# kamisli-icpl/LLICTI

Measured on AMD Instinct MI355X. Metric: MPix/s encode+decode, higher is better.
Workload: dtype f32; 1 GPU; 24x768x512 uniform-noise RGB per GPU, container xauto15 -> xrans20, seed-1337 weights; BASELINE.json configs[2]; batch_per_gpu=24, height=512, width=768, container=xauto15, container_written=xrans20

## Files before the change

### llicti_amd/csrc/cdf.hpp

```cpp
#pragma once

__device__ __forceinline__ StageGeom stage_at(const StageGeom &s, const StageGeom *__restrict__ sv, int b)
{
    if (sv) return sv[b];
    StageGeom r = s;
    r.img_off = (long)b * 3 * s.plane;
    r.par_off = (long)b * LLICTI_PARAM_STRIDE * s.h * s.w;
    r.pair_off = (long)b * s.hc * s.wc;
    return r;
}

__device__ __forceinline__ void clr_range(const int32_t *mm, int clr, int &minv, int &maxv, int &shift)
{
    if (clr == 0) { minv = -127; maxv = 128; shift = 127; }
    else { minv = mm[clr - 1]; maxv = mm[2 + clr - 1]; shift = -minv; }
}

constexpr int kPairsThreads = 256;
__device__ __forceinline__ void cdf_pairs_body(const int16_t *__restrict__ planes, const float *__restrict__ params,
                                               const int32_t *__restrict__ minmax, const StageGeom &s, uint32_t *__restrict__ pairs)
{
    const int b = blockIdx.y;
    const int lane = threadIdx.x & 63, wave = threadIdx.x >> 6;
    const int np = s.h * s.w;
    const int p0 = (blockIdx.x * (blockDim.x >> 6) + wave) * 64;
    if (p0 >= np) return;
    const ParRow par = par_row(params + s.par_off, 0, np, min(p0 + lane, np - 1));
    const int p = p0 + lane;
    const int i = p / s.w, j = p - i * s.w;
    if (p >= np || i >= s.hc || j >= s.wc) return;
    const long n = (long)i * s.wc + j;
    const long off = s.img_off + ((long)(2 * i + s.oi) << s.lvl) * s.W + ((long)(2 * j + s.oj) << s.lvl);
    const int vy = planes[off], vco = planes[off + s.plane], vcg = planes[off + 2 * s.plane];
    const float yv = div255_exact((float)vy), cov = div255_exact((float)vco);
    const int32_t *mm = minmax + 4 * b;
#pragma unroll
    for (int clr = 0; clr < 3; ++clr) {
        int minv, maxv, shift;
        clr_range(mm, clr, minv, maxv, shift);
        const Grid gr = make_grid(minv, maxv);
        const int v = (clr == 0) ? vy : (clr == 1) ? vco : vcg;
        const int sym = v + shift;
        Mix m;
        mix_prepare(par, clr, yv, cov, m);
        const uint32_t lo = cdf_entry(m, gr, sym);
        const uint32_t hi1 = cdf_entry(m, gr, min(sym + 1, gr.Lp - 2));
        const uint32_t hi = (sym == gr.Lp - 2) ? 0u : hi1;
        pairs[(long)clr * s.pair_cs + s.pair_off + n] = (hi << 16) | lo;
    }
}
__global__ __launch_bounds__(kPairsThreads) void cdf_pairs_kernel(const int16_t *__restrict__ planes, const float *__restrict__ params,
                                                        const int32_t *__restrict__ minmax, StageGeom s, const StageGeom *__restrict__ sv,
                                                        uint32_t *__restrict__ pairs)
{
    cdf_pairs_body(planes, params, minmax, stage_at(s, sv, blockIdx.y), pairs);
}
struct PairsBands { const StageGeom *sv[3]; const float *params[3]; uint32_t *pairs[3]; };
__global__ __launch_bounds__(kPairsThreads) void cdf_pairs_bands_kernel(const int16_t *__restrict__ planes, PairsBands a,
                                                              const int32_t *__restrict__ minmax)
{
    const int band = blockIdx.z;
    cdf_pairs_body(planes, a.params[band], minmax, a.sv[band][blockIdx.y], a.pairs[band]);
}

__device__ __forceinline__ Comp row_component(const ParRow &par, const int16_t *__restrict__ planes, long off, long plane, int clr, int mi, float &w)
{
    float a0 = 0.0f, a1 = 0.0f, y = 0.0f, co = 0.0f;
    if (clr == 1) { a0 = par[48 + mi]; y = (float)planes[off] / 255.0f; }
    else if (clr == 2) { a0 = par[48 + 5 + mi]; a1 = par[48 + 10 + mi]; y = (float)planes[off] / 255.0f; co = (float)planes[off + plane] / 255.0f; }
    Comp c = mix_component(clr, par[5 * clr + mi], par[16 + 5 * clr + mi], par[32 + 5 * clr + mi], a0, a1, y, co, w);
    float ssum = w + dpp_row_shl(w, 1);
    ssum = ssum + dpp_row_shl(w, 2);
    ssum = ssum + dpp_row_shl(w, 3);
    ssum = ssum + dpp_row_shl(w, 4);
    c.wn = w / mix_weight_den(__int_as_float(__builtin_amdgcn_readfirstlane(__float_as_int(ssum))));
    return c;
}

constexpr int kTabWaves = 4;

__global__ __launch_bounds__(64 * kTabWaves) void cdf_table_kernel(const int16_t *__restrict__ planes, const float *__restrict__ params,
                                                                   const int32_t *__restrict__ minmax, StageGeom s, int clr,
                                                                   uint16_t *__restrict__ tables, int row_stride,
                                                                   int n0, int cnt, int cap_rows)
{
    const int b = blockIdx.y;
    const int nc = s.hc * s.wc;
    const int lane = threadIdx.x & 63;
    const int wave0 = __builtin_amdgcn_readfirstlane((int)(blockIdx.x * kTabWaves + (threadIdx.x >> 6)));
    const int nwaves = gridDim.x * kTabWaves;
    int minv, maxv, shift;
    clr_range(minmax + 4 * b, clr, minv, maxv, shift);
    const Grid gr = make_grid(minv, maxv);
    const int nblk = (row_stride + 63) >> 6;
    float pt[8];
#pragma unroll
    for (int k = 0; k < 8; ++k) pt[k] = sample_pt(gr, min(64 * k + lane, gr.Lp - 1));
    const float fmin = (float)minv;
    const long img = (long)b * 3 * s.plane;
    const int mi = min(lane, 4);

    constexpr int kTabRun = 8;
    const int n_end = min(nc, n0 + cnt);
    for (int nb = n0 + kTabRun * wave0; nb < n_end; nb += kTabRun * nwaves)
    for (int n = nb; n < min(nb + kTabRun, n_end); ++n) {
        const int i = n / s.wc, j = n - i * s.wc;
        const ParRow par = par_row(params, b, (long)s.h * s.w, (long)i * s.w + j);
        const long off = img + ((long)(2 * i + s.oi) << s.lvl) * s.W + ((long)(2 * j + s.oj) << s.lvl);
        float w;
        const Comp cm = row_component(par, planes, off, s.plane, clr, mi, w);
        const float mu = cm.mu, rsig = cm.rsig, wn = cm.wn;
        const float c = mu * 255.0f - fmin + 0.5f, hw = 9.8994949f * 255.0f * mix_sigma(par[5 * clr + mi]) + 2.0f;
        int lo = -1, hi = 1 << 20;
        if (c - hw > -1.0f && c - hw < 1e6f) lo = (int)(c - hw);
        if (c + hw > -1e6f && c + hw < 1e6f) hi = (int)(c + hw) + 1;
        if (!(c == c) || !(hw == hw)) { lo = -1; hi = 1 << 20; }
        float mu_[5], rs_[5], wn_[5];
        int lo_[5], hi_[5];
#pragma unroll
        for (int k = 0; k < 5; ++k) {
            mu_[k] = __int_as_float(__builtin_amdgcn_readlane(__float_as_int(mu), k));
            rs_[k] = __int_as_float(__builtin_amdgcn_readlane(__float_as_int(rsig), k));
            wn_[k] = __int_as_float(__builtin_amdgcn_readlane(__float_as_int(wn), k));
            lo_[k] = __builtin_amdgcn_readlane(lo, k);
            hi_[k] = __builtin_amdgcn_readlane(hi, k);
        }
        uint16_t *row = tables + ((long)b * cap_rows + (n - n0)) * row_stride;
#pragma unroll
        for (int k = 0; k < 8; ++k) {
            if (k < nblk) {
                const int e = 64 * k + lane;
                const int ec = min(e, gr.Lp - 1);
                const int bmin = (k == 0) ? -20 : 64 * k;
                const int bmax = (64 * k + 63 >= gr.Lp - 1) ? gr.Lp + 19 : 64 * k + 63;
                float acc = 0.0f;
#pragma unroll
                for (int m = 0; m < 5; ++m) {
                    float t;
                    if (bmax <= lo_[m]) t = 0.0f;
                    else if (bmin >= hi_[m]) t = wn_[m];
                    else {
                        const float z = (pt[k] - mu_[m]) * rs_[m];
                        t = wn_[m] * (0.5f * erfc_spec(kNegRsqrt2 * z));
                    }
                    acc = (m == 0) ? t : acc + t;
                }
                const uint32_t v = entry_from_sum(acc, gr.scale, ec);
                if (e < row_stride) row[e] = (uint16_t)((e < gr.Lp) ? v : 0xFFFFu);
            }
        }
    }
}


__global__ __launch_bounds__(64 * kTabWaves) void cdf_anchor_kernel(const int16_t *__restrict__ planes, const float *__restrict__ params,
                                                                    const int32_t *__restrict__ minmax, StageGeom s, int clr,
                                                                    uint8_t *__restrict__ rows, int n0, int cnt, int cap_rows)
{
    const int b = blockIdx.y;
    const int nc = s.hc * s.wc;
    const int lane = threadIdx.x & 63;
    const int wave0 = __builtin_amdgcn_readfirstlane((int)(blockIdx.x * kTabWaves + (threadIdx.x >> 6)));
    const int nwaves = gridDim.x * kTabWaves;
    int minv, maxv, shift;
    clr_range(minmax + 4 * b, clr, minv, maxv, shift);
    const Grid gr = make_grid(minv, maxv);
    const int ec = min(8 * lane, gr.Lp - 1);
    const float pt = sample_pt(gr, ec);
    const long img = (long)b * 3 * s.plane;
    const int mi = min(lane, 4);
    for (int n = n0 + wave0; n < min(nc, n0 + cnt); n += nwaves) {
        const int i = n / s.wc, j = n - i * s.wc;
        const ParRow par = par_row(params, b, (long)s.h * s.w, (long)i * s.w + j);
        const long off = img + ((long)(2 * i + s.oi) << s.lvl) * s.W + ((long)(2 * j + s.oj) << s.lvl);
        float w;
        const Comp cm = row_component(par, planes, off, s.plane, clr, mi, w);
        const float mu = cm.mu, rsig = cm.rsig, wn = cm.wn;
        float acc = 0.0f;
#pragma unroll
        for (int m = 0; m < 5; ++m) {
// ... 14 lines not shown
```

### llicti_amd/csrc/llicti_hip.hip

```cpp
#include <hip/hip_runtime.h>
#include <stdarg.h>
#include <stdint.h>
#include <stdio.h>
#include <stdlib.h>
#include <string.h>
#include <map>
#include <memory>
#include <string>
#include <tuple>
#include <type_traits>
#include <utility>
#include <vector>

#include "../../include/llicti_hip.h"
#include "numerics.hpp"

using namespace llicti;

#include "common.hpp"
#include "lift.hpp"
#include "likelihood.hpp"
#include "band_cnn.hpp"
#include "cdf.hpp"
#include "ac_coder.hpp"
// ... 890 lines not shown
    TensorNorm nm{};
    PlanDev *target = nullptr;
    uint8_t *target_ws = nullptr;
};

static int resolve_sink(DecodeSink &k, int B, const int *Hs, const int *Ws, int reduce, const int *rv = nullptr)
{
    switch (k.kind) {
    case DecodeSink::Interleaved: {
        std::vector<int> Hw(B), Ww(B);
        for (int b = 0; b < B; ++b) { const int r = rv ? rv[b] : reduce; Hw[b] = reduced_dim(Hs[b], r); Ww[b] = reduced_dim(Ws[b], r); }
        return resolve_pixels("decode_images_px", B, Hw.data(), Ww.data(), k.px.fmt, k.px.off, k.px.pitch, k.pix);
    }
    case DecodeSink::Tensor:
        return resolve_tensor("decode_images_tensor", B, Hs, Ws, reduce, k.tensor, k.wins, k.nm, rv);
    case DecodeSink::Resized:
        return resolve_resize("decode_images_tensor_resized", B, Hs, Ws, reduce, k.resize, k.wins, k.nm, rv);
    case DecodeSink::Views:
        return resolve_views("decode_images_tensor_views", B, Hs, Ws, reduce, k.views, k.groups, k.nm, rv);
    default:
        return 0;
    }
}

template <typename F> static void with_tensor_type(int dtype, F &&f)
{
    if (dtype == LLICTI_T_F32) f(float());
    else if (dtype == LLICTI_T_F16) f(_Float16());
    else f(bf16_bits());
}
template <typename S> static S arg_slice(const std::vector<uint32_t> &words, int k, int first, int n)
{
    S a;
    memset(&a, 0, sizeof a);
    memcpy(a.w, words.data() + (size_t)k * first, (size_t)k * n * sizeof(uint32_t));
    return a;
}

static int launch_sink(llicti_ctx *c, PlanDev *pd, const DecodeSink &k, uint8_t *ws, hipStream_t s, int reduce, const RvCall *rv = nullptr)
{
    const int *rtab = rv ? rv->d_r() : nullptr;
    const Plan &p = pd->p;
    const int B = p.B;
    const int16_t *planes = (const int16_t *)(ws + p.off_planes);
    const int32_t *status = (const int32_t *)(ws + p.off_status);
    const ImgGeo *d_img = pd->dev<ImgGeo>(p.d_img);
    if (k.kind == DecodeSink::Transcode) return 0;
    ProfSpan span(c, PROF_MISC, s);
    switch (k.kind) {
    case DecodeSink::Tensor: {
        const TensorArgs &t = k.tensor;
        const int gx = (int)std::min<long>(((long)t.Ho * ((t.Wo + 3) / 4) + 255) / 256, 1024);
        for (int b0 = 0; b0 < B; b0 += kTensorWinMax) {
            const int nb = std::min(kTensorWinMax, B - b0);
            const TensorWins tw = arg_slice<TensorWins>(k.wins, 1, b0, nb);
            with_tensor_type(t.dtype, [&](auto e) {
                using T = decltype(e);
                unlift_tensor_kernel<T><<<dim3(gx, nb), 256, 0, s>>>(planes, (T *)k.d_out, reduce, t.Ho, t.Wo, b0, tw, k.nm, status, kStatusHead, c->d_status,
                                                                    c->d_img_status, d_img, rtab);
            });
        }
        break;
    }
    case DecodeSink::Resized: {
        const ResizeArgs &t = k.resize;
        const int tiles_x = (t.Wo + kResizeTileW - 1) / kResizeTileW, tiles_y = (t.Ho + kResizeTileH - 1) / kResizeTileH;
        for (int b0 = 0; b0 < B; b0 += kResizeBoxMax) {
            const int nb = std::min(kResizeBoxMax, B - b0);
            const ResizeBoxes bx = arg_slice<ResizeBoxes>(k.wins, 2, b0, nb);
            with_tensor_type(t.dtype, [&](auto e) {
                using T = decltype(e);
                unlift_resize_tensor_kernel<T><<<dim3(tiles_x * tiles_y, nb), 256, 0, s>>>(planes, (T *)k.d_out, reduce, t.Ho, t.Wo, b0, tiles_x, t.antialias, bx, k.nm,
                                                                                          status, kStatusHead, c->d_status, c->d_img_status, d_img, rtab);
            });
        }
        break;
    }
    case DecodeSink::Views: {
        int latch_n = B;
        for (const ViewGroupOut &g : k.groups) {
            const int tiles_x = (g.Wo + kResizeTileW - 1) / kResizeTileW, tiles_y = (g.Ho + kResizeTileH - 1) / kResizeTileH;
            for (int v0 = 0; v0 < g.n; v0 += kViewMax) {
                const int nv = std::min(kViewMax, g.n - v0);
                const ViewSlice vs = arg_slice<ViewSlice>(g.words, 3, v0, nv);
                with_tensor_type(g.dtype, [&](auto e) {
                    using T = decltype(e);
                    unlift_views_tensor_kernel<T><<<dim3(tiles_x * tiles_y, nv), 256, 0, s>>>(planes, (T *)g.d_out, reduce, g.Ho, g.Wo, v0, tiles_x, g.antialias, vs, k.nm,
                                                                                             status, kStatusHead, c->d_status, c->d_img_status, d_img, latch_n, rtab);
                });
                latch_n = 0;
            }
        }
        break;
    }
    case DecodeSink::Interleaved: {
        const int gx = (int)std::min<long>(((rv ? rv->q.pix_units : p.pix_units) + 255) / 256, 1024);
        if (rv) unlift_px_kernel<<<dim3(gx, B), 256, 0, s>>>(planes, k.d_out, 0, status, kStatusHead, c->d_status, c->d_img_status, d_img, rv->d_red(), rv->d_pix(), rtab);
        else unlift_px_kernel<<<dim3(gx, B), 256, 0, s>>>(planes, k.d_out, reduce, status, kStatusHead, c->d_status, c->d_img_status, d_img,
                                                          reduce > 0 ? pd->dev<RedGeo>(p.d_red) : nullptr, pd->dev<PixGeo>(p.d_pix));
        break;
    }
    default:
        if (rv) {
            unlift_reduced_kernel<<<dim3((unsigned)((rv->q.max_rplane + 255) / 256), B), 256, 0, s>>>(planes, k.d_out, 0, status, kStatusHead, c->d_status,
                                                                                                      c->d_img_status, d_img, rv->d_red(), rtab);
        } else if (reduce > 0) {
            long max_rplane = 0;
            for (const RedGeo &rg : p.red) max_rplane = std::max(max_rplane, (long)rg.Hr * rg.Wr);
            unlift_reduced_kernel<<<dim3((unsigned)((max_rplane + 255) / 256), B), 256, 0, s>>>(planes, k.d_out, reduce, status, kStatusHead, c->d_status,
                                                                                                c->d_img_status, d_img, pd->dev<RedGeo>(p.d_red));
        } else {
            const int gx = (int)std::min<long>((p.max_plane + 255) / 256, 1024);
            unlift_kernel<<<dim3(gx, B), 256, 0, s>>>(planes, p.max_plane, k.d_out, status, kStatusHead, c->d_status, c->d_img_status, d_img);
        }
    }
    HIPCHK(hipGetLastError());
    return 0;
}

static int decode_stages(llicti_ctx *c, PlanDev *pd, const uint8_t *d_in, size_t in_stride, const int32_t *d_seg_len, uint8_t *ws, hipStream_t s, int reduce,
                         const DecodeSink &sink, const RvCall *rv = nullptr)
{
    const Plan &p = pd->p;
    const int B = p.B, M = p.M, Q = p.Q;
    int16_t *planes = (int16_t *)(ws + p.off_planes);
    float *fplanes = (float *)(ws + p.off_fplanes);
    int32_t *mm = (int32_t *)(ws + p.off_minmax);
    int32_t *status = (int32_t *)(ws + p.off_status);
    float *params = (float *)(ws + p.off_params);
    uint8_t *slots = ws + p.off_slots;
    uint8_t *tables = ws + p.off_tables;
    uint32_t *acstate = (uint32_t *)(ws + p.off_acstate);
    int32_t *slot_len = (int32_t *)(ws + p.off_slot_len);
    const ImgGeo *d_img = pd->dev<ImgGeo>(p.d_img);
    const Geom *d_geo = pd->dev<Geom>(p.d_geo);
    const StageGeom *d_sg = pd->dev<StageGeom>(p.d_sg);
    const long *d_rslot_off = pd->dev<long>(p.d_rslot_off);
    const StreamRef *d_sref = pd->dev<StreamRef>(p.d_sref);
    const int NS = p.nstreams;
    const TileRef *d_tiles = p.uniform ? nullptr : pd->dev<TileRef>(p.d_tiles);

    zero_words_kernel<<<(kStatusHead + B + 255) / 256, 256, 0, s>>>(status, kStatusHead + B);
    uint32_t *rstate = (uint32_t *)(ws + p.off_rstate);
    uint32_t *rpos = (uint32_t *)(ws + p.off_rpos);
    uint32_t *rtail = (uint32_t *)(ws + p.off_rtail);
    {
        ProfSpan span(c, PROF_MISC, s);
        header_read_kernel<<<B, 256, 0, s>>>(d_in, (long)in_stride, d_seg_len, d_img, planes, fplanes, mm, status);
        if (M == 0) {
            const int st0 = first_stage(p.nlev);
            unpack_kernel<<<dim3(LLICTI_NSTREAMS - st0, B), 256, 0, s>>>(d_in, (long)in_stride, d_seg_len, B, slots, pd->dev<long>(p.d_slot_off), pd->dev<int32_t>(p.d_slot_cap), slot_len, status, st0);
        } else {
            const StageGeom *sglv = d_sg + (size_t)(0 * 3 + 2) * B;
            rans_unpack_kernel<<<NS, 256, 0, s>>>(d_in, (long)in_stride, d_seg_len, d_sref, 2 + Q * RansGeo<1>::kPayBytes,
                                                  slots, d_rslot_off, p.rslot_cap, rpos, status, Q == 4 ? 4 : 2);
            if (Q == 4) rans_init_kernel<4><<<NS, 64, 0, s>>>(slots, d_rslot_off, d_sref, rstate, rpos, rtail, status, sglv);
            else if (Q == 2) rans_init_kernel<2><<<NS, 64, 0, s>>>(slots, d_rslot_off, d_sref, rstate, rpos, rtail, status, sglv);
            else rans_init_kernel<1><<<NS, 64, 0, s>>>(slots, d_rslot_off, d_sref, rstate, rpos, rtail, status, sglv);
        }
    }
    if (rv && M == 0) return fail(LLICTI_EINVAL, "decode_images: per-image reduces need rANS containers");
    for (int lvl = p.nlev - 1; lvl >= reduce; --lvl) {
        const Geom &g = p.geo[(size_t)lvl * B];
        const Geom *gv = (p.uniform && !rv) ? nullptr : d_geo + (size_t)lvl * B;
        const int NS = rv ? rv->q.s_n[lvl] : p.nstreams;
        const int *act = rv ? rv->dev<int>(rv->q.d_streams) + rv->q.s_off[lvl] : nullptr;
        if (NS == 0 && M > 0) continue;
        for (int band = 0; band < 3; ++band) {
            const TileRun *run = rv ? &rv->q.run[lvl * 3 + band] : &p.run[lvl * 3 + band];
            const TileRef *tl = rv ? rv->dev<TileRef>(rv->q.d_tiles) + run->off : d_tiles ? d_tiles + run->off : nullptr;
            if (int rc = launch_band_params(c, fplanes, g, band, params, s, gv, tl, run)) return rc;
            const StageGeom *sgv = d_sg + (size_t)(lvl * 3 + band) * B;
            if (M > 0) {
                const int last = (lvl == 0 && band == 2) ? 1 : 0;
                {
                ProfSpan span(c, PROF_RANS_STAGE, s);
                if (Q == 4) {
                    rans_decode_stage_lane_kernel<4><<<NS, 256, 0, s>>>(params, sgv, d_sref, slots, d_rslot_off, p.rslot_cap, rstate, rpos, rtail, planes, fplanes, mm, last, status, c->d_phi_lut, act);
                } else if (Q == 2) {
                    rans_decode_stage_pair_kernel<<<NS, 64 * kRansWaves, 0, s>>>(params, sgv, d_sref, c->d_phi_lut, slots, d_rslot_off, p.rslot_cap, rstate, rpos, rtail, planes, fplanes, mm, last, status, act);
                } else {
                    rans_decode_stage_kernel<<<NS, 64 * kRansWaves, 0, s>>>(params, sgv, d_sref, c->d_phi_lut, slots, d_rslot_off, p.rslot_cap, rstate, rpos, rtail, planes, fplanes, mm, last, status, act);
                }
                }
                if (last) {
                    ProfSpan span(c, PROF_RANS_TAIL, s);
                    if (Q == 4) rans_tail_kernel<4><<<NS, 64 * (1 + kTailAhead) * kTailChains<4>, 0, s>>>(params, sgv, d_sref, rstate, rpos, rtail, planes, fplanes, mm, status, slots, d_rslot_off, act);
                    else if (Q == 2) rans_tail_kernel<2><<<NS, 64 * (1 + kTailAhead), 0, s>>>(params, sgv, d_sref, rstate, rpos, rtail, planes, fplanes, mm, status, slots, d_rslot_off, act);
                    else rans_tail_kernel<1><<<NS, 64 * (1 + kTailAhead), 0, s>>>(params, sgv, d_sref, rstate, rpos, rtail, planes, fplanes, mm, status, slots, d_rslot_off, act);
                }
            }
            if (M == 0) {
                const StageGeom sg = make_stage(g, band);
                const long nc = (long)sg.hc * sg.wc;
                const int C = ac_chunks(nc);
                const long rows = ac_chunk_rows(nc);
                hipStream_t q[3] = { s, c->sub[1], c->sub[2] };
                if (C > 1) {
                    HIPCHK(hipEventRecord(c->ev_ac_band, s));
                    HIPCHK(hipStreamWaitEvent(q[1], c->ev_ac_band, 0));
                    HIPCHK(hipStreamWaitEvent(q[2], c->ev_ac_band, 0));
                }
                for (int ch = 0; ch < C; ++ch) {
                    const long n0 = (long)ch * rows, cnt = std::min(rows, nc - n0);
                    for (int clr = 0; clr < 3; ++clr) {
                        hipStream_t qs = (C > 1) ? q[clr] : s;
                        if (C > 1 && clr > 0) HIPCHK(hipStreamWaitEvent(qs, c->ev_ac[clr - 1][ch], 0));
                        ProfSpan span(c, PROF_AC, qs);
                        const bool anchors = ac_use_anchors(B, c->ac_anchor_min_batch);
                        const int row_stride = (clr == 0) ? 264 : 512;
                        uint8_t *tab = tables + (size_t)clr * B * p.ac_cap_rows * (anchors ? (size_t)kAnchorRow : (size_t)1024);
                        if (anchors) { if (int rc = launch_cdf_anchors(planes, params, mm, g, band, clr, tab, n0, cnt, p.ac_cap_rows, qs)) return rc; }
                        else if (int rc = launch_cdf_table(planes, params, mm, g, band, clr, (uint16_t *)tab, row_stride, n0, cnt, p.ac_cap_rows, qs)) return rc;
                        const int st = stage_index(lvl, band, clr);
                        DecOut o;
                        memset(&o, 0, sizeof o);
                        o.planes = planes; o.fplanes = fplanes; o.minmax = mm; o.sg = sg; o.clr = clr;
                        o.len = slot_len + (size_t)st * B;
                        const long in_stride_slots = p.slot_cap[(size_t)st * B];
                        AcChunk ck = { (int)n0, (int)cnt, (int)nc, (int)p.ac_cap_rows, acstate + (size_t)clr * B * 8 };
                        if (anchors) ac_decode_anchor_kernel<<<B, 64, 0, qs>>>(tab, slots + p.slot_off[(size_t)st * B], in_stride_slots, ck, o);
                        else ac_decode_kernel<<<B, 64, 0, qs>>>((const uint16_t *)tab, 0, row_stride, slots + p.slot_off[(size_t)st * B], in_stride_slots, ck, o);
                        if (C > 1 && clr < 2) HIPCHK(hipEventRecord(c->ev_ac[clr][ch], qs));
                    }
                }
                if (C > 1) {
                    for (int k = 1; k < 3; ++k) {
                        HIPCHK(hipEventRecord(c->ev_ac_end[k - 1], q[k]));
                        HIPCHK(hipStreamWaitEvent(s, c->ev_ac_end[k - 1], 0));
                    }
                }
            }
            if (sink.kind == DecodeSink::Transcode) {
                const Plan &q = sink.target->p;
                const int k = lvl * 3 + band;
                ProfSpan span(c, PROF_PAIRS, s);
                cdf_pairs_kernel<<<dim3((unsigned)((q.lev_maxpos[lvl] + kPairsThreads - 1) / kPairsThreads), B), kPairsThreads, 0, s>>>(
                    planes, params, mm, q.sg[(size_t)k * B], sink.target->dev<StageGeom>(q.d_sg) + (size_t)k * B,
                    (uint32_t *)(sink.target_ws + q.off_pairs) + q.pair_base[k]);
                HIPCHK(hipGetLastError());
            }
        }
    }
    return launch_sink(c, pd, sink, ws, s, reduce, rv);
}

static int reserve_img_status(llicti_ctx *c, int B)
{
    c->img_status_n = 0;
    if (c->img_status_cap < B) {
        ++c->n_device_sync; ++c->n_device_alloc;
        HIPCHK(hipDeviceSynchronize());
        if (c->d_img_status) { (void)hipFree(c->d_img_status); c->d_img_status = nullptr; c->img_status_cap = 0; }
        const int cap = std::max(B, 64);
        HIPCHK(hipMalloc(&c->d_img_status, (size_t)cap * sizeof(int32_t)));
        c->img_status_cap = cap;
    }
    return 0;
}

static int decode_batch(llicti_ctx *c, const uint8_t *d_in, size_t in_stride, const int32_t *d_seg_len, int B, const int *Hs, const int *Ws,
                        const int *modes, int n_modes, void *d_workspace, size_t workspace_bytes, const size_t *rgb_off, void *stream, int reduce, DecodeSink sink,
                        const int *reduces = nullptr)
{
    const bool own_out = sink.kind == DecodeSink::Views;
    if (!c || !d_in || !d_seg_len || !d_workspace || (!sink.d_out && !own_out)) return fail(LLICTI_EINVAL, "decode_images: null pointer");
    if (reduce < 0 || reduce > c->nlev) return fail(LLICTI_EINVAL, "decode_images: reduce = %d (a %d-level model decodes at reduce 0 .. %d)", reduce, c->nlev, c->nlev);
    if (check_dims_v(B, Hs, Ws)) return LLICTI_EINVAL;
    int ME = 0;
    std::vector<int> Ms;
    if (int rc = resolve_modes("decode_images", modes, n_modes, B, &ME, Ms)) return rc;
    if (int rc = check_model(c->nlev, "decode_images", ME, Ms)) return rc;
    if (int rc = check_stream_bits("decode_images", c->nlev, B, Hs, Ws, ME, Ms)) return rc;
    if (reduces) if (int rc = admit_reduces("decode_images", B, reduces, c->nlev, ME)) return rc;
    if (int rc = resolve_sink(sink, B, Hs, Ws, reduce, reduces)) return rc;
    if (int rc = check_source_modes("decode_images", "container", ME)) return rc;
    for (int b = 0; b < 3; ++b) if (!c->have[b]) return fail(LLICTI_ENOWEIGHTS, "band %d weights not set", b);
    DeviceGuard guard(c);
    hipStream_t s = (hipStream_t)stream;
    PlanDev *pd = nullptr;
    if (reduces) { if (int rc = get_plan(c, B, Hs, Ws, nullptr, ME, modes_ptr(Ms), s, &pd)) return rc; }
    else if (int rc = get_plan(c, B, Hs, Ws, rgb_off, ME, modes_ptr(Ms), s, &pd, reduce, sink.kind == DecodeSink::Interleaved ? &sink.pix : nullptr)) return rc;
    PlanUse use{ pd, s };
    const Plan &p = pd->p;
    if (!p.uniform && p.M == 0) return fail(LLICTI_EINVAL, "decode_images: a batch of mixed sizes needs a rANS container (the reference-format container codes equal sizes per call)");
    if (int rc = check_in_stride("decode_images", p.nlev, B, Hs, Ws, in_stride)) return rc;
    if (workspace_bytes < p.total)
        return fail(LLICTI_ENOSPACE, "decode_images: workspace %zu < %zu", workspace_bytes, p.total);

    if (int rc = reserve_img_status(c, B)) return rc;
    RvCall rv;
    if (reduces) {
        rv.c = c; rv.s = s;
        build_reduce_schedule(rv.q, p, reduces, sink.kind == DecodeSink::Planar ? rgb_off : nullptr, c->n_cu, c->cnn_tile_rows,
                              sink.kind == DecodeSink::Interleaved ? &sink.pix : nullptr);
        if (int rc = rv.upload()) return rc;
        reduce = rv.q.rmin;
    }
    CallScope call(c, s);
    if (int rc = decode_stages(c, pd, d_in, in_stride, d_seg_len, (uint8_t *)d_workspace, s, reduce, sink, reduces ? &rv : nullptr)) return rc;
    c->img_status_n = B;
    return LLICTI_OK;
}
static DecodeSink planar_sink(uint8_t *d_rgb) { DecodeSink k; k.d_out = d_rgb; return k; }

extern "C" int llicti_decode_images_v(llicti_ctx *c, const uint8_t *d_in, size_t in_stride, const int32_t *d_seg_len,
                                      int B, const int *Hs, const int *Ws, int mode, void *d_workspace, size_t workspace_bytes,
                                      uint8_t *d_rgb, const size_t *rgb_off, void *stream)
{
    return decode_batch(c, d_in, in_stride, d_seg_len, B, Hs, Ws, &mode, 1, d_workspace, workspace_bytes, rgb_off, stream, 0, planar_sink(d_rgb));
}
// ... 412 lines not shown
```

### llicti_amd/csrc/rans_coder.hpp

```cpp
#pragma once
#include <type_traits>

#include "prove_symbol.hpp"


__device__ __forceinline__ int lanes_below(uint64_t mask)
{
    return (int)__builtin_amdgcn_mbcnt_hi((uint32_t)(mask >> 32), __builtin_amdgcn_mbcnt_lo((uint32_t)mask, 0u));
}

__device__ __forceinline__ int wave_incl_scan(int v)
{
    v += __builtin_amdgcn_update_dpp(0, v, 0x111, 0xF, 0xF, true);
    v += __builtin_amdgcn_update_dpp(0, v, 0x112, 0xF, 0xF, true);
    v += __builtin_amdgcn_update_dpp(0, v, 0x114, 0xF, 0xF, true);
    v += __builtin_amdgcn_update_dpp(0, v, 0x118, 0xF, 0xF, true);
    v += __builtin_amdgcn_update_dpp(0, v, 0x142, 0xA, 0xF, false);
    v += __builtin_amdgcn_update_dpp(0, v, 0x143, 0xC, 0xF, false);
    return v;
}

__device__ __forceinline__ int rans_emit_bits(uint32_t x, uint32_t freq)
{
    if (freq >= 0x10000u) return 0;
// ... 287 lines not shown
                const uint32_t lo = v & 0xFFFFu;
                uint32_t hi = v >> 16;
                if (hi == 0) hi = 0x10000u;
                uint32_t freq = hi - lo;
                if (freq == 0 || hi < lo) { bad = 1; freq = 1; }
                if (T == 0) xt = freq << 15;
                const int nb = (T == 0) ? 0 : rans_emit_bits(xt, freq);
                if (tb + nb + 32 > GEO::kPayBits) { full = true; break; }
                acc |= (uint64_t)(xt & ((1u << nb) - 1u)) << accn;
                accn += nb;
                tb += nb;
                if (accn >= 32) {
                    if (tid == 0) sh_pay[wdw] = (uint32_t)acc;
                    ++wdw; acc >>= 32; accn -= 32;
                }
                xt = rans_push(xt >> nb, lo, freq);
                ++T;
            }
            raw = rawn;
        }
        acc |= (uint64_t)xt << accn;
        if (tid == 0) { sh_pay[wdw] = (uint32_t)acc; if (accn > 0) sh_pay[wdw + 1] = (uint32_t)(acc >> 32); }
        __syncthreads();
    }
    uint32_t x = (1u << 31) | lds_get_bits(sh_pay, kRansStateBits * tid, kRansStateBits);
    const int tail_from = cnt - T;

    int bp = alen - GEO::kPayBits, wbase = 0;
    int par = 0;
    struct Stg { const uint32_t *pp; int n, K, lim; };
    auto stage_of = [&](int st) -> Stg {
        if (st < 0) return Stg{ pairs, 1, 0, 0 };
        const StreamDesc d = desc[(long)st * B + b];
        const int nchunks = (d.n + L - 1) / L;
        return Stg{ pairs + d.pair_off, max(d.n, 1), (nchunks <= m) ? 0 : (nchunks - m + M - 1) / M,
                    (st == LLICTI_NSTREAMS - 1) ? tail_from : 0x7FFFFFFF };
    };
    auto fetch_of = [&](const Stg &g, int k) -> uint32_t { return g.pp[min(L * (m + max(k, 0) * M) + tid, g.n - 1)]; };
    Stg sg_cur = stage_of(LLICTI_NSTREAMS - 1);
    uint32_t a0 = fetch_of(sg_cur, sg_cur.K - 1), a1 = fetch_of(sg_cur, sg_cur.K - 2), a2 = fetch_of(sg_cur, sg_cur.K - 3), a3 = fetch_of(sg_cur, sg_cur.K - 4);
    uint32_t b0 = fetch_of(sg_cur, sg_cur.K - 5), b1 = fetch_of(sg_cur, sg_cur.K - 6), b2 = fetch_of(sg_cur, sg_cur.K - 7), b3 = fetch_of(sg_cur, sg_cur.K - 8);
    for (int st = LLICTI_NSTREAMS - 1; st >= 0; --st) {
        const Stg d = sg_cur;
        const Stg sg_nxt = stage_of(st - 1);
        const uint32_t n0 = fetch_of(sg_nxt, sg_nxt.K - 1), n1 = fetch_of(sg_nxt, sg_nxt.K - 2), n2 = fetch_of(sg_nxt, sg_nxt.K - 3), n3 = fetch_of(sg_nxt, sg_nxt.K - 4);
        const uint32_t n4 = fetch_of(sg_nxt, sg_nxt.K - 5), n5 = fetch_of(sg_nxt, sg_nxt.K - 6), n6 = fetch_of(sg_nxt, sg_nxt.K - 7), n7 = fetch_of(sg_nxt, sg_nxt.K - 8);
        const int K = d.K;
        const int lim = d.lim;
        auto fetch = [&](int k) -> uint32_t { return fetch_of(d, k); };
        auto round4 = [&](int k, uint32_t raw0, uint32_t raw1, uint32_t raw2, uint32_t raw3) {
            const uint32_t raws[4] = { raw0, raw1, raw2, raw3 };
            uint32_t fld[4];
            int nbs[4];
#pragma unroll
            for (int j = 0; j < 4; ++j) {
                const int kk = k - j;
                const int n = L * (m + kk * M) + tid;
                const bool active = kk >= 0 && n < d.n && L * kk + tid < lim;
                const uint32_t v = active ? raws[j] : 0u;
                const uint32_t lo = v & 0xFFFFu;
                uint32_t hi = v >> 16;
                hi = (hi == 0) ? 0x10000u : hi;
                uint32_t freq = hi - lo;
                const bool wrong = (freq == 0) | (hi < lo);
                bad = wrong ? 1 : bad;
                freq = wrong ? 1u : freq;
                const int nb = rans_emit_bits(x, freq);
                nbs[j] = nb;
                fld[j] = x & ((1u << nb) - 1u);
                const uint32_t xn = rans_push(x >> nb, lo, freq);
                x = active ? xn : x;
            }
            int incl[4], total[4];
#pragma unroll
            for (int j = 0; j < 4; ++j) { incl[j] = wave_incl_scan(nbs[j]); total[j] = __builtin_amdgcn_readlane(incl[j], 63); }
            int below[4] = { 0, 0, 0, 0 }, step_total[4] = { total[0], total[1], total[2], total[3] };
            if constexpr (Q > 1) {
                if (lane == 0) *reinterpret_cast<int4 *>(&sh_tot[par][wq][0]) = make_int4(total[0], total[1], total[2], total[3]);
                lds_barrier();
#pragma unroll
                for (int j = 0; j < 4; ++j) step_total[j] = 0;
#pragma unroll
                for (int q2 = 0; q2 < Q; ++q2) {
                    const int4 t4 = *reinterpret_cast<const int4 *>(&sh_tot[par][q2][0]);
                    const int t[4] = { t4.x, t4.y, t4.z, t4.w };
#pragma unroll
                    for (int j = 0; j < 4; ++j) { step_total[j] += t[j]; below[j] += (q2 > wq) ? t[j] : 0; }
                }
                par ^= 1;
            }
            while (bp - 32 * wbase >= 32 * kFlush) {
                const int slot_i = (wbase + tid) & (kWin - 1);
                if (wbase + kFlush <= cap_dw) out32[wbase + tid] = sh_win[slot_i]; else bad = 2;
                sh_win[slot_i] = 0;
                wbase += kFlush;
            }
#pragma unroll
            for (int j = 0; j < 4; ++j) {
                const int pos = bp + below[j] + (total[j] - incl[j]);
                const int sh = pos & 31;
                atomicOr(&sh_win[(pos >> 5) & (kWin - 1)], fld[j] << sh);
                atomicOr(&sh_win[((pos >> 5) + 1) & (kWin - 1)], (uint32_t)(((uint64_t)fld[j] << sh) >> 32));
                bp += step_total[j];
            }
        };
        for (int k = K - 1; k >= 0; k -= 8) {
            round4(k, a0, a1, a2, a3);
            a0 = fetch(k - 8); a1 = fetch(k - 9); a2 = fetch(k - 10); a3 = fetch(k - 11);
            if (k - 4 >= 0) round4(k - 4, b0, b1, b2, b3);
            b0 = fetch(k - 12); b1 = fetch(k - 13); b2 = fetch(k - 14); b3 = fetch(k - 15);
        }
        a0 = n0; a1 = n1; a2 = n2; a3 = n3; b0 = n4; b1 = n5; b2 = n6; b3 = n7;
        sg_cur = sg_nxt;
    }
    __syncthreads();
    if constexpr (kSeeded<Q>) {
        if (tid == 0) {
            const uint32_t f10 = (uint32_t)((T + kRansTailBlock - 1) / kRansTailBlock) | ((uint32_t)tail_single << 8) | (1u << 9);
            const int sh = bp & 31;
            atomicOr(&sh_win[(bp >> 5) & (kWin - 1)], f10 << sh);
            atomicOr(&sh_win[((bp >> 5) + 1) & (kWin - 1)], (uint32_t)(((uint64_t)f10 << sh) >> 32));
        }
        bp += 10;
        __syncthreads();
    }
    const int nbytes = (bp + 7) >> 3;
    sh_pay[tid] = 0;
    __syncthreads();
    lds_or_bits(sh_pay, kRansStateBits * tid, 16, x & 0xFFFFu);
    lds_or_bits(sh_pay, kRansStateBits * tid + 16, kRansStateBits - 16, (x >> 16) & 0x7FFFu);
    __syncthreads();
    const int ndw = (nbytes >> 2) - wbase;
    const bool over = (nbytes >> 2) + 1 > cap_dw;
    if (over) bad = 2;
    else {
        for (int t = tid; t < ndw; t += 64 * Q) out32[wbase + t] = sh_win[(wbase + t) & (kWin - 1)];
        if (tid < (nbytes & 3)) slot[4 + (nbytes & ~3) + tid] = (uint8_t)(sh_win[(wbase + ndw) & (kWin - 1)] >> (8 * tid));
        uint8_t *fs = slot + 4 + nbytes;
        for (int t = tid; t < GEO::kPayBytes; t += 64 * Q) fs[t] = (uint8_t)(sh_pay[t >> 2] >> (8 * (t & 3)));
    }
    if (tid == 0) {
        if constexpr (kSeeded<Q>) {
            rinfo[2 * sidx] = 4; rinfo[2 * sidx + 1] = (bad == 2) ? 0 : nbytes + GEO::kPayBytes;
        } else {
            const int t16 = (T & 0x7FF) | ((8 * nbytes - bp) << 11);
            slot[2] = (uint8_t)(t16 & 0xFF); slot[3] = (uint8_t)(t16 >> 8);
            rinfo[2 * sidx] = 2; rinfo[2 * sidx + 1] = (bad == 2) ? 0 : 2 + nbytes + GEO::kPayBytes;
        }
    }
    if (bad) atomicExch(&status[0], bad == 1 ? LLICTI_EFORMAT : LLICTI_ENOSPACE);
}

template <int Q>
__global__ __launch_bounds__(64) void rans_init_kernel(const uint8_t *__restrict__ slots, const long *__restrict__ rslot_off,
                                                       const StreamRef *__restrict__ sref, uint32_t *__restrict__ rstate, uint32_t *__restrict__ rpos,
                                                       uint32_t *__restrict__ rtail, int32_t *status, const StageGeom *__restrict__ sglv)
{
    using GEO = RansGeo<Q>;
    const int sidx = blockIdx.x, lane = threadIdx.x;
    const uint8_t *slot = slots + rslot_off[sidx];
    const int n = (int)rpos[sidx];
    bool bad = false;
    int T = 0, single = 0, cur = 0, nbytes;
    if constexpr (kSeeded<Q>) {
        nbytes = n - GEO::kPayBytes;
        const uint8_t *reg = slot + 4;
        const int lastb = reg[nbytes - 1];
        const int top = 8 * (nbytes - 1) + 31 - __clz(lastb | 1);
        if (lastb == 0 || top < 9) bad = true;
        else {
            const int p0 = top - 9;
            const uint32_t w = (uint32_t)reg[p0 >> 3] | ((uint32_t)reg[(p0 >> 3) + 1] << 8) | ((uint32_t)reg[min((p0 >> 3) + 2, nbytes - 1)] << 16);
            const uint32_t f9 = (w >> (p0 & 7)) & 0x1FFu;
            const StreamRef sr_ = sref[sidx];
            const StageGeom sgl = sglv[sr_.b];
            T = min(kRansTailBlock * (int)(f9 & 0xFFu), rans_stream_count(sgl.hc * sgl.wc, sr_.m, sr_.M, GEO::kLanes));
            single = (int)(f9 >> 8);
            cur = p0;
        }
    } else {
        const int t16 = slot[2] | (slot[3] << 8);
        T = t16 & 0x7FF;
        nbytes = n - 2 - GEO::kPayBytes;
        const int pad = (t16 >> 11) & 7;
        if ((t16 >> 14) || nbytes < 0 || (nbytes == 0 && pad)) { bad = true; T = 0; nbytes = max(nbytes, 0); }
        else if (pad && (slot[4 + nbytes - 1] >> (8 - pad))) { bad = true; T = 0; }
        cur = bad ? 0 : 8 * nbytes - pad;
    }
    const uint8_t *fs = slot + 4 + nbytes;
#pragma unroll
    for (int qq = 0; qq < Q; ++qq) {
        const int bpos = kRansStateBits * (64 * qq + lane);
        uint64_t w = 0;
#pragma unroll
        for (int k = 0; k < 5; ++k) w |= (uint64_t)fs[min((bpos >> 3) + k, GEO::kPayBytes - 1)] << (8 * k);
        rstate[((long)sidx * Q + qq) * 64 + lane] = (1u << 31) | ((uint32_t)(w >> (bpos & 7)) & 0x7FFFFFFFu);
    }
    if (lane == 0) { rpos[sidx] = (uint32_t)cur; rtail[sidx] = (uint32_t)T | ((uint32_t)single << 16); }
    if (bad && lane == 0) flag_image(status, sref[sidx].b, LLICTI_EFORMAT);
}

constexpr int kRansWaves = 4;

__device__ __forceinline__ float dpp_sum5(float tA, float tB)
{
    float acc = tA + dpp_row_shl(tA, 1);
    acc = acc + dpp_row_shl(tA, 2);
    acc = acc + dpp_row_shl(tA, 3);
    acc = acc + dpp_row_shl(tB, 3);
    return acc;
}
__device__ __forceinline__ float quad_lane0(float v)
{
    return __int_as_float(__builtin_amdgcn_update_dpp(0, __float_as_int(v), 0x00, 0xF, 0xF, true));
}

template <int J>
__device__ __forceinline__ float quad_bcast(float v)
{
    return __int_as_float(__builtin_amdgcn_update_dpp(0, __float_as_int(v), J * 0x55, 0xF, 0xF, true));
}

__device__ __forceinline__ uint32_t group_cdf_entry(const Comp &A, const Comp &B, const Grid &g, int i)
{
    const float pt = sample_pt(g, i);
    const float tA = mix_term(A.wn, A.mu, A.rsig, pt);
    const float tB = mix_term(B.wn, B.mu, B.rsig, pt);
    return entry_from_sum(dpp_sum5(tA, tB), g.scale, i);
}

struct CompFast { float c1, c0, wh, wn; };
__device__ __forceinline__ CompFast comp_fast(const Comp &c)
{
    CompFast f;
    f.c1 = (kNegRsqrt2 * 1.2011224087864498f) * c.rsig;
    f.c0 = -c.mu * f.c1;
    f.wh = 0.5f * c.wn;
    f.wn = c.wn;
    return f;
}
__device__ __forceinline__ float term_fast(const CompFast &c, float pt)
{
    const float x = __builtin_fmaf(pt, c.c1, c.c0);
    const float a = __builtin_fabsf(x);
    const float u = __builtin_amdgcn_rcpf(__builtin_fmaf(0.3275911f / 1.2011224087864498f, a, 1.0f));
    float p = __builtin_fmaf(1.061405429f, u, -1.453152027f);
    p = __builtin_fmaf(p, u, 1.421413741f);
    p = __builtin_fmaf(p, u, -0.284496736f);
    p = __builtin_fmaf(p, u, 0.254829592f);
    const float E = ((p * u) * __builtin_amdgcn_exp2f(-(a * a))) * c.wh;
    return (x < 0.0f) ? c.wn - E : E;
}
struct CompLut { float c1, c0, wn; };
__device__ __forceinline__ CompLut comp_lut(const Comp &c)
{
    constexpr float kS = kPhiLutN / (2.0f * (float)kPhiLutZ);
    CompLut f;
    f.c1 = c.rsig * kS;
    f.c0 = __builtin_fmaf(-c.mu, f.c1, (float)kPhiLutZ * kS);
    f.wn = c.wn;
    return f;
}
__device__ __forceinline__ float term_lut(const CompLut &c, float pt, const float2 *lut)
{
    const float u = __builtin_amdgcn_fmed3f(__builtin_fmaf(pt, c.c1, c.c0), 0.0f, (float)kPhiLutN - 0.0009765625f);
    const float2 e2 = lut[(uint32_t)u];
    return c.wn * __builtin_fmaf(e2.y, __builtin_amdgcn_fractf(u), e2.x);
}
__device__ __forceinline__ int group_cdf_entry_fast(const CompFast &A, const CompFast &B, float fbase, float scale, int i)
{
    const float pt = div255_exact(fbase + (float)i);
    return (int)__builtin_rintf(dpp_sum5(term_fast(A, pt), term_fast(B, pt)) * scale) + i;
}

__global__ __launch_bounds__(64 * kRansWaves) void rans_decode_stage_kernel(const float *__restrict__ params, const StageGeom *__restrict__ sgv, const StreamRef *__restrict__ sref,
                                                               const float2 *__restrict__ phi_lut,
                                                               const uint8_t *__restrict__ slots, const long *__restrict__ rslot_off,
                                                               int rslot_cap, uint32_t *__restrict__ rstate, uint32_t *__restrict__ rpos,
                                                               const uint32_t *__restrict__ rtail,
                                                               int16_t *__restrict__ planes, float *__restrict__ fplanes,
                                                               const int32_t *__restrict__ minmax, int last_stage, int32_t *status,
                                                               const int *__restrict__ act = nullptr)
{
    __shared__ uint32_t sh_res[2][64][2];
    __shared__ float2 sh_lut[kPhiLutN];
    const int sidx = act ? act[blockIdx.x] : (int)blockIdx.x;
    const StreamRef sr_ = sref[sidx];
    const int b = sr_.b, m = sr_.m, M = sr_.M;
    const int lane = threadIdx.x & 63, wave = threadIdx.x >> 6;
    const StageGeom sg = sgv[b];
    const int nc = sg.hc * sg.wc;
    const int nchunks = (nc + 63) >> 6;
    if (nchunks <= m) return;
    for (int j = threadIdx.x; j < kPhiLutN; j += 64 * kRansWaves) sh_lut[j] = phi_lut[j];
    __syncthreads();
    const int K = (nchunks - m + M - 1) / M;
    uint32_t x = rstate[(long)sidx * 64 + lane];
    int bcur = (int)rpos[sidx];
    const uint32_t *bitw = reinterpret_cast<const uint32_t *>(slots + rslot_off[sidx] + 4);
    const int max_dw = (rslot_cap - 4) >> 2;
    int wtop = max(64, (((bcur + 31) >> 5) + 63) & ~63);
    auto load_dw = [&](int d0) -> uint32_t { return bitw[min(max(d0 + lane, 0), max_dw - 1)]; };
    uint32_t winA = load_dw(wtop - 64), winB = load_dw(wtop - 128);
    int badx = 0;
    auto pass = [&](auto tag) {
    constexpr int clr = decltype(tag)::value;
    const int tail_from = (last_stage && clr == 2) ? rans_stream_count(nc, m, M, 64) - (int)(rtail[sidx] & 0xFFFFu) : 0x7FFFFFFF;
    int minv, maxv, shift;
    clr_range(minmax + 4 * b, clr, minv, maxv, shift);
    const Grid gr = make_grid(minv, maxv);
    const int max_symbol = gr.Lp - 2;
    const float fbase = (float)minv - 0.5f;
    const long img = sg.img_off;
    const int mA = lane & 3;
    const int gsym = 16 * wave + (lane >> 2);
    const int gbit = lane & ~3;
    const bool head = (mA == 0);
    struct Raw { float sgA, muA, wkA, a0A, a1A, sgB, muB, wkB, a0B, a1B, y, co; long off; bool on; };
    auto fetch = [&](int k) -> Raw {
        Raw r;
        const int n = min(64 * (m + k * M) + gsym, nc - 1);
        const int i = div_wc(sg, n), j = n - i * sg.wc;
        const ParRow32 par = par_row32(params + sg.par_off, 0, (long)sg.h * sg.w, (long)i * sg.w + j);
        r.off = img + ((long)(2 * i + sg.oi) << sg.lvl) * sg.W + ((long)(2 * j + sg.oj) << sg.lvl);
        r.sgA = par[5 * clr + mA]; r.muA = par[16 + 5 * clr + mA]; r.wkA = par[32 + 5 * clr + mA];
        r.sgB = par[5 * clr + 4];  r.muB = par[16 + 5 * clr + 4];  r.wkB = par[32 + 5 * clr + 4];
        r.a0A = r.a1A = r.a0B = r.a1B = r.y = r.co = 0.0f;
        if constexpr (clr == 1) { r.a0A = par[48 + mA]; r.a0B = par[48 + 4]; r.y = fplanes[r.off]; }
        else if constexpr (clr == 2) {
            r.a0A = par[48 + 5 + mA]; r.a1A = par[48 + 10 + mA]; r.a0B = par[48 + 5 + 4]; r.a1B = par[48 + 10 + 4];
            r.y = fplanes[r.off]; r.co = fplanes[r.off + sg.plane];
        }
        r.on = (k < K) && (64 * (m + k * M) + gsym) < nc && (64 * k + gsym) < tail_from;
        return r;
    };
    Raw cur = fetch(0);
    for (int k = 0; k < K; ++k) {
        const int chunk0 = 64 * (m + k * M);
        Raw nxt = fetch(min(k + 1, K - 1));
        const uint32_t slot = (uint32_t)__builtin_amdgcn_ds_bpermute(4 * gsym, (int)x) & 0xFFFFu;
        {
            if (cur.on) {
                const long off = cur.off;
                float wA, wB;
                Comp A = mix_component<clr>(cur.sgA, cur.muA, cur.wkA, cur.a0A, cur.a1A, cur.y, cur.co, wA);
                Comp B = mix_component<clr>(cur.sgB, cur.muB, cur.wkB, cur.a0B, cur.a1B, cur.y, cur.co, wB);
                const float den = mix_weight_den(quad_lane0(dpp_sum5(wA, wB)));
                A.wn = wA / den;
                B.wn = wB / den;

                const CompLut Af = comp_lut(A), Bf = comp_lut(B);
                CompLut F0, F1, F2, F3;
// ... 700 lines not shown
            if (wb >= 0) np = __builtin_popcountll((ballot64((uint32_t)wv <= slot) & 0xFFFull) | (wb == 0 ? 1ull : 0ull));
            uint32_t vlo, vhi;
            if (np >= 1 && np <= 11) {
                vlo = (uint32_t)__builtin_amdgcn_readlane(wv, np - 1);
                vhi = (uint32_t)__builtin_amdgcn_readlane(wv, np);
            } else {
                const float mu = sh_cmp[buf][sl][mc], rsig = sh_cmp[buf][sl][5 + mc], wn = sh_cmp[buf][sl][10 + mc];
                const int e1 = sh_e1[buf][sl][lane];
                auto entry_at = [&](int idx) -> uint32_t {
                    const float pt = sample_pt(gr, min(idx, gr.Lp - 1));
                    const float term = mix_term(wn, mu, rsig, pt);
                    const int g0 = 4 * 5 * min(we, 11);
                    const float a0 = __int_as_float(__builtin_amdgcn_ds_bpermute(g0, __float_as_int(term)));
                    const float a1 = __int_as_float(__builtin_amdgcn_ds_bpermute(g0 + 4, __float_as_int(term)));
                    const float a2 = __int_as_float(__builtin_amdgcn_ds_bpermute(g0 + 8, __float_as_int(term)));
                    const float a3 = __int_as_float(__builtin_amdgcn_ds_bpermute(g0 + 12, __float_as_int(term)));
                    const float a4 = __int_as_float(__builtin_amdgcn_ds_bpermute(g0 + 16, __float_as_int(term)));
                    const float acc = (((a0 + a1) + a2) + a3) + a4;
                    return (idx <= max_symbol) ? entry_from_sum(acc, gr.scale, idx) : 0x10000u;
                };
                const uint64_t p1 = ballot64(lane == 0 || (8 * lane <= max_symbol && e1 <= (int)slot));
                wb = max(8 * (__builtin_popcountll(p1) - 1) - 2, 0);
                uint32_t ent = entry_at(wb + we);
                const uint64_t pw12 = ballot64(mc == 0 && we < 12 && wb + we <= max_symbol && (ent <= slot || wb + we == 0));
                np = __builtin_popcountll(pw12);
                if (np == 0 || np == 12) {
                    int lo = 0, hi = max_symbol + 1;
                    while (hi - lo > 1) {
                        const int stp = (hi - lo + 12) / 13;
                        const int pi = min(lo + stp * (min(we, 11) + 1), hi - 1);
                        const uint32_t e = entry_at(pi);
                        const uint64_t pb = ballot64(mc == 0 && we < 12 && e <= slot);
                        const int k = __builtin_popcountll(pb);
                        const int nlo = (k > 0) ? min(lo + stp * k, hi - 1) : lo;
                        const int nhi = (k < 12) ? min(lo + stp * (k + 1), hi - 1) : hi;
                        lo = nlo; hi = nhi;
                    }
                    wb = lo;
                    ent = entry_at(wb + we);
                    np = 1;
                }
                vlo = (uint32_t)__builtin_amdgcn_readlane((int)ent, 5 * (np - 1));
                vhi = (uint32_t)__builtin_amdgcn_readlane((int)ent, 5 * np);
            }
            vsym = (lane == i) ? wb + np - 1 - shift : vsym;
            xt = (vhi - vlo) * (xt >> 16) + slot - vlo;
            if constexpr (kSeeded<Q>) {
                int nb = __clz((int)xt);
                if (nch == 2) {
                    const int avail = chain ? tc - 32 : alen - 32 - tc;
                    if (nb > 16 || avail < nb) { bad = true; nb = max(min(nb, min(avail, 16)), 0); }
                    if (chain) tc -= nb;
                    xt = ((xt << nb) | take_bits(tc, nb)) | (1u << 31);
                    if (!chain) tc += nb;
                } else {
                    const int avail = a_end - tc;
                    if (nb > avail) nb = max(avail, 0);
                    else if (nb > 16) bad = true;
                    if (nb > 16) { bad = true; nb = 16; }
                    xt = (xt << nb) | take_bits(tc, nb);
                    tc += nb;
                }
            } else if (SA * r + i == T - 1) bad = bad || xt != (vhi - vlo) << 15;
            else {
                int nb = __clz((int)xt);
                if (nb > 16 || tc < nb) { bad = true; nb = max(min(nb, min(tc, 16)), 0); }
                tc -= nb;
                xt = ((xt << nb) | take_bits(tc, nb)) | (1u << 31);
            }
        }
        if (lane < SA && SA * r + lane < T) {
            const long off = sh_off[buf][chain * kTailAhead + lane];
            planes[off + 2 * sg.plane] = (int16_t)vsym;
            fplanes[off + 2 * sg.plane] = div255_exact((float)vsym);
        }
        lds_barrier();
    }
    if constexpr (kSeeded<Q>) {
        const uint32_t A = (uint32_t)(max_symbol + 1), v = (nch == 2) ? (xt & 0x7FFFFFFFu) : xt;
        bad = bad || (live && (nch == 2 ? v >= pw : (v >= A || tc != a_end)));
        uint32_t div = 1;
        for (int e = 0; e < min(lane, sn); ++e) div *= A;
        const int dg = (lane < sn) ? (int)((v / div) % A) : 0;
        const int j = chain * sn + lane;
        if (live && lane < sn && j < NS) {
            const long pp = pixel_of(j);
            const int pi = (int)(pp >> 32), pj = (int)(uint32_t)pp;
            const long off = img + ((long)(2 * pi + sg.oi) << sg.lvl) * sg.W + ((long)(2 * pj + sg.oj) << sg.lvl);
            const int pv = dg - shift;
            planes[off + 2 * sg.plane] = (int16_t)pv;
            fplanes[off + 2 * sg.plane] = div255_exact((float)pv);
        }
        bad = bad || ballot64(live && lane < sn && j >= NS && dg != 0) != 0;
        if (lane == 0) sh_cur[chain] = tc;
        lds_barrier();
        if (chain == 0 && nch == 2) {
            const int ca = sh_cur[0], cb = sh_cur[1];
            uint32_t nz = 0;
            for (int d = lane; d < GEO::kPayDw + kSpillDw; d += 64) {
                const int lo = max(ca, 32 * d), hi = min(cb, 32 * d + 32);
                if (lo < hi) nz |= sh_pay[d] & ((hi - lo == 32) ? 0xFFFFFFFFu : (((1u << (hi - lo)) - 1u) << (lo - 32 * d)));
            }
            bad = bad || ca > cb || ballot64(nz != 0) != 0;
        }
        if (bad && lane == 0) flag_image(status, b, LLICTI_EFORMAT);
    } else {
        if (T == 0) bad = bad || xt != (1u << 31);
        if ((bad || tc != 0) && lane == 0) flag_image(status, b, LLICTI_EFORMAT);
    }
}

__global__ __launch_bounds__(256) void rans_pack_kernel(const uint8_t *__restrict__ slots, const long *__restrict__ rslot_off,
                                                        const int32_t *__restrict__ rinfo, const StreamRef *__restrict__ sref, const ImgGeo *__restrict__ iv,
                                                        uint8_t *__restrict__ out, long out_stride, int32_t *__restrict__ seg_len, int32_t *status,
                                                        const unsigned long long *__restrict__ ssum, const StreamDesc *__restrict__ desc, int B)
{
    const StreamRef sr_ = sref[blockIdx.x];
    const int b = sr_.b, m = sr_.m, M = image_stream_count(ssum, iv, desc, B, sr_.b, sr_.M), s0 = sr_.sbase;
    const int hdr_bytes = iv[b].hdr_bytes;
    if (ssum && iv[b].Mlo && m == 0 && threadIdx.x == 0) {
        uint8_t *oh = out + (long)b * out_stride;
        const int pf = (iv[b].padint & 0x3FF) | (M << 10);
        oh[15] = (uint8_t)(pf & 0xFF); oh[16] = (uint8_t)((pf >> 8) & 0xFF);
    }
    if (m >= M) {
        if (threadIdx.x == 0) seg_len[(long)b * LLICTI_NSEG + 4 + m] = 0;
        return;
    }
    const int G = rans_group(M), sg = m / G;
    long dst = hdr_bytes + (G > 1 ? 4L * G * (sg + 1) : 0);
    for (int k = 0; k < m; ++k) dst += rinfo[2 * (s0 + k) + 1];
    const int n = rinfo[2 * (s0 + m) + 1];
    if (dst + n > out_stride) { if (threadIdx.x == 0) atomicExch(&status[0], LLICTI_ENOSPACE); return; }
    const uint8_t *src = slots + rslot_off[s0 + m] + rinfo[2 * (s0 + m)];
    uint8_t *o = out + (long)b * out_stride + dst;
    block_copy_bytes(o, src, n);
    if (threadIdx.x == 0) {
        if (G == 1) seg_len[(long)b * LLICTI_NSEG + 4 + m] = n;
        else if (m % G == 0) {
            uint8_t *tab = o - 4 * G;
            int tot = 4 * G;
            for (int k = 0; k < G; ++k) {
                const int len = rinfo[2 * (s0 + m + k) + 1];
                tab[4 * k] = (uint8_t)(len & 0xFF); tab[4 * k + 1] = (uint8_t)((len >> 8) & 0xFF);
                tab[4 * k + 2] = (uint8_t)((len >> 16) & 0xFF); tab[4 * k + 3] = (uint8_t)((len >> 24) & 0xFF);
                tot += len;
            }
            seg_len[(long)b * LLICTI_NSEG + 4 + sg] = tot;
        }
        if (m == 0) for (int k = 4 + M / G; k < LLICTI_NSEG; ++k) seg_len[(long)b * LLICTI_NSEG + k] = 0;
    }
}

__global__ __launch_bounds__(256) void rans_unpack_kernel(const uint8_t *__restrict__ in, long in_stride, const int32_t *__restrict__ seg_len,
                                                          const StreamRef *__restrict__ sref, int min_stream, uint8_t *__restrict__ slots, const long *__restrict__ rslot_off,
                                                          int rslot_cap, uint32_t *__restrict__ rpos, int32_t *status, int stream_off)
{
    const StreamRef sr_ = sref[blockIdx.x];
    const int b = sr_.b, m = sr_.m, M = sr_.M, s0 = sr_.sbase;
    const int G = rans_group(M), sg = m / G;
    const int32_t *sl = seg_len + (long)b * LLICTI_NSEG;
    long src = 0;
    bool bad = false;
    for (int k = 0; k < 4 + sg; ++k) {
        const int v = sl[k];
        if (v < 0 || v > in_stride) bad = true;
        src += v;
        if (src < 0 || src > in_stride) { bad = true; src = 0; }
    }
    int n = sl[4 + sg];
    if (G > 1) {
        const int seg_n = n;
        if (bad || seg_n < 4 * G || src + seg_n > in_stride) { bad = true; n = 0; }
        else {
            const uint8_t *tab = in + (long)b * in_stride + src;
            long off = 4L * G, tot = 4L * G;
            for (int k = 0; k < G; ++k) {
                const long len = (long)tab[4 * k] | ((long)tab[4 * k + 1] << 8) | ((long)tab[4 * k + 2] << 16) | ((long)tab[4 * k + 3] << 24);
                if (len < min_stream || len > seg_n) bad = true;
                if (k < m % G) off += len;
                if (k == m % G) n = (int)min(len, (long)seg_n);
                tot += len;
            }
            if (tot != seg_n) bad = true;
            src += off;
        }
    }
    uint8_t *o = slots + rslot_off[s0 + m] + stream_off;
    if (bad || n < min_stream || n + 4 + 64 > rslot_cap || src + n > in_stride) {
        if (threadIdx.x == 0) flag_image(status, b, LLICTI_EFORMAT);
        n = min_stream;
        for (int t = threadIdx.x; t < n; t += blockDim.x) o[t] = 0;
    } else {
        const uint8_t *p = in + (long)b * in_stride + src;
        block_copy_bytes(o, p, n);
    }
    const int padded = min(rslot_cap - stream_off, n + 64);
    for (int t = n + threadIdx.x; t < padded; t += blockDim.x) o[t] = 0;
    if (threadIdx.x == 0) rpos[s0 + m] = (uint32_t)n;
}
```

Before: 453.6 MPix/s.

## Fuse rANS stream init into unpack kernel and preload pair params into registers

The per-stream rANS state initialisation moves into the unpack kernel: after a block barrier, the first wave parses the stream it just copied. This drops one kernel launch and a round-trip of rpos through global memory. Separately, the CDF pairs kernel now loads all parameter channels up front into a register array with nontemporal loads, instead of reading them lazily. That adds register pressure and may lower occupancy.

```diff
diff --git a/llicti_amd/csrc/cdf.hpp b/llicti_amd/csrc/cdf.hpp
--- a/llicti_amd/csrc/cdf.hpp
+++ b/llicti_amd/csrc/cdf.hpp
@@ -17,6 +17,17 @@
 }
 
 constexpr int kPairsThreads = 256;
+struct PairsPar {
+    float v[64];
+    __device__ __forceinline__ float operator[](int ch) const { return v[ch]; }
+    __device__ __forceinline__ void load(const ParRow &r)
+    {
+#pragma unroll
+        for (int ch = 0; ch < 63; ++ch)
+            if (ch % 16 != 15) v[ch] = __builtin_nontemporal_load(r.img + (long)ch * r.stride + r.pos);
+        __builtin_amdgcn_sched_barrier(0);
+    }
+};
 __device__ __forceinline__ void cdf_pairs_body(const int16_t *__restrict__ planes, const float *__restrict__ params,
                                                const int32_t *__restrict__ minmax, const StageGeom &s, uint32_t *__restrict__ pairs)
 {
@@ -25,7 +36,8 @@
     const int np = s.h * s.w;
     const int p0 = (blockIdx.x * (blockDim.x >> 6) + wave) * 64;
     if (p0 >= np) return;
-    const ParRow par = par_row(params + s.par_off, 0, np, min(p0 + lane, np - 1));
+    PairsPar par;
+    par.load(par_row(params + s.par_off, 0, np, min(p0 + lane, np - 1)));
     const int p = p0 + lane;
     const int i = p / s.w, j = p - i * s.w;
     if (p >= np || i >= s.hc || j >= s.wc) return;
diff --git a/llicti_amd/csrc/llicti_hip.hip b/llicti_amd/csrc/llicti_hip.hip
--- a/llicti_amd/csrc/llicti_hip.hip
+++ b/llicti_amd/csrc/llicti_hip.hip
@@ -1066,11 +1066,10 @@
             unpack_kernel<<<dim3(LLICTI_NSTREAMS - st0, B), 256, 0, s>>>(d_in, (long)in_stride, d_seg_len, B, slots, pd->dev<long>(p.d_slot_off), pd->dev<int32_t>(p.d_slot_cap), slot_len, status, st0);
         } else {
             const StageGeom *sglv = d_sg + (size_t)(0 * 3 + 2) * B;
-            rans_unpack_kernel<<<NS, 256, 0, s>>>(d_in, (long)in_stride, d_seg_len, d_sref, 2 + Q * RansGeo<1>::kPayBytes,
-                                                  slots, d_rslot_off, p.rslot_cap, rpos, status, Q == 4 ? 4 : 2);
-            if (Q == 4) rans_init_kernel<4><<<NS, 64, 0, s>>>(slots, d_rslot_off, d_sref, rstate, rpos, rtail, status, sglv);
-            else if (Q == 2) rans_init_kernel<2><<<NS, 64, 0, s>>>(slots, d_rslot_off, d_sref, rstate, rpos, rtail, status, sglv);
-            else rans_init_kernel<1><<<NS, 64, 0, s>>>(slots, d_rslot_off, d_sref, rstate, rpos, rtail, status, sglv);
+            const int min_stream = 2 + Q * RansGeo<1>::kPayBytes, stream_off = Q == 4 ? 4 : 2;
+            if (Q == 4) rans_unpack_kernel<4><<<NS, 256, 0, s>>>(d_in, (long)in_stride, d_seg_len, d_sref, min_stream, slots, d_rslot_off, p.rslot_cap, rpos, status, stream_off, rstate, rtail, sglv);
+            else if (Q == 2) rans_unpack_kernel<2><<<NS, 256, 0, s>>>(d_in, (long)in_stride, d_seg_len, d_sref, min_stream, slots, d_rslot_off, p.rslot_cap, rpos, status, stream_off, rstate, rtail, sglv);
+            else rans_unpack_kernel<1><<<NS, 256, 0, s>>>(d_in, (long)in_stride, d_seg_len, d_sref, min_stream, slots, d_rslot_off, p.rslot_cap, rpos, status, stream_off, rstate, rtail, sglv);
         }
     }
     if (rv && M == 0) return fail(LLICTI_EINVAL, "decode_images: per-image reduces need rANS containers");
diff --git a/llicti_amd/csrc/rans_coder.hpp b/llicti_amd/csrc/rans_coder.hpp
--- a/llicti_amd/csrc/rans_coder.hpp
+++ b/llicti_amd/csrc/rans_coder.hpp
@@ -463,14 +463,10 @@
 }
 
 template <int Q>
-__global__ __launch_bounds__(64) void rans_init_kernel(const uint8_t *__restrict__ slots, const long *__restrict__ rslot_off,
-                                                       const StreamRef *__restrict__ sref, uint32_t *__restrict__ rstate, uint32_t *__restrict__ rpos,
-                                                       uint32_t *__restrict__ rtail, int32_t *status, const StageGeom *__restrict__ sglv)
+__device__ __forceinline__ void rans_init_stream(const uint8_t *slot, int n, int sidx, const StreamRef &sr_, int lane, uint32_t *__restrict__ rstate,
+                                                 uint32_t *__restrict__ rpos, uint32_t *__restrict__ rtail, int32_t *status, const StageGeom *__restrict__ sglv)
 {
     using GEO = RansGeo<Q>;
-    const int sidx = blockIdx.x, lane = threadIdx.x;
-    const uint8_t *slot = slots + rslot_off[sidx];
-    const int n = (int)rpos[sidx];
     bool bad = false;
     int T = 0, single = 0, cur = 0, nbytes;
     if constexpr (kSeeded<Q>) {
@@ -483,7 +479,6 @@
             const int p0 = top - 9;
             const uint32_t w = (uint32_t)reg[p0 >> 3] | ((uint32_t)reg[(p0 >> 3) + 1] << 8) | ((uint32_t)reg[min((p0 >> 3) + 2, nbytes - 1)] << 16);
             const uint32_t f9 = (w >> (p0 & 7)) & 0x1FFu;
-            const StreamRef sr_ = sref[sidx];
             const StageGeom sgl = sglv[sr_.b];
             T = min(kRansTailBlock * (int)(f9 & 0xFFu), rans_stream_count(sgl.hc * sgl.wc, sr_.m, sr_.M, GEO::kLanes));
             single = (int)(f9 >> 8);
@@ -508,7 +503,7 @@
         rstate[((long)sidx * Q + qq) * 64 + lane] = (1u << 31) | ((uint32_t)(w >> (bpos & 7)) & 0x7FFFFFFFu);
     }
     if (lane == 0) { rpos[sidx] = (uint32_t)cur; rtail[sidx] = (uint32_t)T | ((uint32_t)single << 16); }
-    if (bad && lane == 0) flag_image(status, sref[sidx].b, LLICTI_EFORMAT);
+    if (bad && lane == 0) flag_image(status, sr_.b, LLICTI_EFORMAT);
 }
 
 constexpr int kRansWaves = 4;
@@ -1515,9 +1510,11 @@
     }
 }
 
+template <int Q>
 __global__ __launch_bounds__(256) void rans_unpack_kernel(const uint8_t *__restrict__ in, long in_stride, const int32_t *__restrict__ seg_len,
                                                           const StreamRef *__restrict__ sref, int min_stream, uint8_t *__restrict__ slots, const long *__restrict__ rslot_off,
-                                                          int rslot_cap, uint32_t *__restrict__ rpos, int32_t *status, int stream_off)
+                                                          int rslot_cap, uint32_t *__restrict__ rpos, int32_t *status, int stream_off,
+                                                          uint32_t *__restrict__ rstate, uint32_t *__restrict__ rtail, const StageGeom *__restrict__ sglv)
 {
     const StreamRef sr_ = sref[blockIdx.x];
     const int b = sr_.b, m = sr_.m, M = sr_.M, s0 = sr_.sbase;
@@ -1560,5 +1557,6 @@
     }
     const int padded = min(rslot_cap - stream_off, n + 64);
     for (int t = n + threadIdx.x; t < padded; t += blockDim.x) o[t] = 0;
-    if (threadIdx.x == 0) rpos[s0 + m] = (uint32_t)n;
-}
+    __syncthreads();
+    if (threadIdx.x < 64) rans_init_stream<Q>(o - stream_off, n, s0 + m, sr_, (int)threadIdx.x, rstate, rpos, rtail, status, sglv);
+}
```

New measurement: 453.1 MPix/s. Within noise of the previous version (-0.1%).
